# facebookresearch/AudioDec

Hardware: NVIDIA H100
Metric: 48 kHz audio samples/s, encode+quantize+lookup+decode (% HBM roofline in `roofline`) (higher is better)
Workload: dtype f32

## Files before the change

### audiodec_b200/_lib.py

```python
from __future__ import annotations

import ctypes
import os

_HERE = os.path.dirname(os.path.abspath(__file__))
LIB_PATH = os.environ.get("ADEC_LIB_PATH") or os.path.join(_HERE, "lib", "libaudiodec_b200.so")
MAX_STAGES = 8

c_int, c_float, c_void_p, c_char_p = ctypes.c_int, ctypes.c_float, ctypes.c_void_p, ctypes.c_char_p
c_int64 = ctypes.c_int64
_I8 = c_int * MAX_STAGES


class AdecConfig(ctypes.Structure):
    _fields_ = [
        ("model_type", c_int),
        ("input_channels", c_int), ("output_channels", c_int), ("encode_channels", c_int), ("decode_channels", c_int),
        ("code_dim", c_int), ("codebook_num", c_int), ("codebook_size", c_int),
        ("n_enc", c_int), ("enc_ratios", _I8), ("enc_strides", _I8),
        ("n_dec", c_int), ("dec_ratios", _I8), ("dec_strides", _I8),
        ("bias", c_int),
        ("in_channels", c_int), ("out_channels", c_int), ("channels", c_int), ("kernel_size", c_int),
        ("n_up", c_int), ("upsample_scales", _I8), ("upsample_kernel_sizes", _I8),
        ("resblock_kernel_size", c_int),
# ... 9 lines not shown


MODEL_SYMAD, MODEL_HIFIGAN, MODEL_SYMAD_DECODER = 0, 1, 2


class AdecTestOp(ctypes.Structure):
    _fields_ = [
        ("kind", c_int), ("Cin", c_int), ("Cout", c_int), ("K", c_int), ("stride", c_int), ("dil", c_int), ("groups", c_int),
        ("shared_in", c_int), ("pre_act", c_int), ("slope", c_float), ("out_nct", c_int), ("post_tanh", c_int),
        ("w", c_void_p), ("w2", c_void_p), ("bias", c_void_p), ("mean", c_void_p), ("scale", c_void_p),
        ("compute_dtype", c_int),
    ]


TEST_CONV, TEST_RU, TEST_CONVTR, TEST_STEM, TEST_HEAD = 0, 1, 2, 3, 4
TEST_REC = 9

SYMBOLS = {
    "adec_create": (c_int, [ctypes.POINTER(AdecConfig), c_int, ctypes.POINTER(c_void_p)]),
    "adec_destroy": (None, [c_void_p]),
    "adec_last_error": (c_char_p, [c_void_p]),
    "adec_set_tensor": (c_int, [c_void_p, c_char_p, c_void_p, ctypes.POINTER(c_int64), c_int]),
    "adec_finalize": (c_int, [c_void_p]),
    "adec_n_streams": (c_int, [c_void_p]),
    "adec_set_streams": (c_int, [c_void_p, c_int]),
    "adec_reset": (c_int, [c_void_p, c_void_p]),
    "adec_encode": (c_int, [c_void_p, c_void_p, c_int, c_int, c_void_p, c_void_p]),
    "adec_quantize": (c_int, [c_void_p, c_void_p, c_int, c_int, c_void_p, c_void_p]),
    "adec_quantize_ex": (c_int, [c_void_p, c_void_p, c_int, c_int, c_void_p, c_void_p, c_void_p, c_void_p]),
    "adec_quantize_forward": (c_int, [c_void_p, c_void_p, c_int, c_int, c_void_p, c_void_p, c_void_p]),
    "adec_zq_moments": (c_int, [c_void_p, c_void_p, ctypes.POINTER(c_int), c_int, c_void_p, c_void_p, c_void_p]),
# ... 66 lines not shown
```

### audiodec_b200/csrc/adec.cu

```cuda
#include <cuda_runtime.h>

#include <algorithm>
#include <cmath>
#include <cstdarg>
#include <cstdio>
#include <cstring>
#include <map>
#include <memory>
#include <set>
#include <string>
#include <vector>

#include "../../include/audiodec_b200.h"
#include "kernels.cuh"
#include "wg_conv.cuh"
#include <cuda_fp16.h>
#include <cuda_bf16.h>

using namespace adec;

namespace {
thread_local std::string g_create_error;

std::string fmt(const char* f, ...) {
// ... 46 lines not shown
const ConvKernelCfg kConvKernels[] = {
    ADEC_PLAIN(32), ADEC_PLAIN(64), ADEC_PLAIN(96), ADEC_PLAIN(128), ADEC_PLAIN(256),
    {32, 32, 256, 32, true, launch_conv<32, 32, 256, 32, true>},
    {64, 64, 128, 32, true, launch_conv<64, 64, 128, 32, true>},
    {128, 128, 64, 16, true, launch_conv<128, 128, 64, 16, true>},
    {256, 256, 64, 8, true, launch_conv<256, 256, 64, 8, true>},
};

const ConvKernelCfg* find_conv_kernel(int CW, int CO, bool fuse) {
    for (const auto& k : kConvKernels)
        if (k.CW == CW && k.CO == CO && k.fuse == fuse) return &k;
    return nullptr;
}

typedef cudaError_t (*TcPersistFn)(const ConvArgs&, int, int, int, int, int, cudaStream_t);
template <int NT, bool F, int PRE, int PREC, bool BST, bool VL, bool PAIR = false>
cudaError_t launch_wg(const ConvArgs& a, int n_xtiles, int n_ytiles, int n_tiles, int n_ctas, int smem_bytes, cudaStream_t s) {
    static bool configured[64] = {false};
    int dev = 0;
    cudaGetDevice(&dev);
    auto kern = wg_conv_kernel<NT, F, PRE, PREC, BST, VL, PAIR>;
    constexpr int kMaxDyn = 227 * 1024;
    if (dev < 64 && !configured[dev]) {
        cudaError_t e = cudaFuncSetAttribute(kern, cudaFuncAttributeMaxDynamicSharedMemorySize, kMaxDyn);
        if (e != cudaSuccess) return e;
        configured[dev] = true;
    }
    if (smem_bytes > kMaxDyn) return cudaErrorInvalidConfiguration;
    static const bool pdl = [] { const char* e = getenv("ADEC_PDL"); return !e || atoi(e) != 0; }();
    cudaLaunchConfig_t cfg{};
    cfg.gridDim = dim3((unsigned)n_ctas);
    cfg.blockDim = dim3((unsigned)WgCfg<NT, PREC>::THREADS);
    cfg.dynamicSmemBytes = (size_t)smem_bytes;
    cfg.stream = s;
    cudaLaunchAttribute attr[1];
    attr[0].id = cudaLaunchAttributeProgrammaticStreamSerialization;
    attr[0].val.programmaticStreamSerializationAllowed = 1;
    cfg.attrs = attr;
    cfg.numAttrs = pdl ? 1 : 0;
    return cudaLaunchKernelEx(&cfg, kern, a, n_xtiles, n_ytiles, n_tiles);
}
typedef size_t (*TcSmemFn)(int, bool, bool);
typedef int (*TcWbufFn)(int, bool, bool);
template <int NT, bool F, int PRE, int PREC, bool BST>
constexpr TcPersistFn pair_fn() {
    if constexpr (NT == 32 && F && PREC == PREC_F16 && !BST) return launch_wg<NT, F, PRE, PREC, BST, false, true>;
    else return nullptr;
}
struct TcKernelCfg { int NT; bool fuse; int pre, prec; bool bst; int tap_bytes; TcPersistFn pfn, pfn_vl, pfn_pair; TcSmemFn smem; TcWbufFn n_wbuf; };
#define ADEC_TC1(NT, F, PRE, PREC, BST) \
    {NT, F, PRE, PREC, BST, WgCfg<NT, PREC>::TAP_BYTES, launch_wg<NT, F, PRE, PREC, BST, false>, launch_wg<NT, F, PRE, PREC, BST, true>, \
     pair_fn<NT, F, PRE, PREC, BST>(), WgCfg<NT, PREC>::smem_bytes, WgCfg<NT, PREC>::n_wbuf}
#define ADEC_TC_FP32(NT, PREC) \
    ADEC_TC1(NT, true, ACT_ELU, PREC, false), ADEC_TC1(NT, false, ACT_NONE, PREC, false), ADEC_TC1(NT, false, ACT_ELU, PREC, false), \
    ADEC_TC1(NT, false, ACT_LRELU, PREC, false), ADEC_TC1(NT, false, ACT_NORM, PREC, false)
#define ADEC_TC_BF16(NT, BST) \
    ADEC_TC1(NT, false, ACT_NONE, PREC_BF16, BST), ADEC_TC1(NT, false, ACT_LRELU, PREC_BF16, BST), ADEC_TC1(NT, false, ACT_NORM, PREC_BF16, BST), \
    ADEC_TC1(NT, true, ACT_ELU, PREC_BF16, BST), ADEC_TC1(NT, false, ACT_ELU, PREC_BF16, BST)
#define ADEC_TC(NT) ADEC_TC_FP32(NT, PREC_F16), ADEC_TC_FP32(NT, PREC_TF32), ADEC_TC_BF16(NT, false), ADEC_TC_BF16(NT, true)
const TcKernelCfg kTcKernels[] = {ADEC_TC(128), ADEC_TC(64), ADEC_TC(32)};

const TcKernelCfg* find_tc_kernel(int NT, bool fuse, int pre, int prec, bool bst) {
    for (const auto& k : kTcKernels)
        if (k.NT == NT && k.fuse == fuse && k.pre == pre && k.prec == prec && k.bst == bst) return &k;
    return nullptr;
}

// ... 60 lines not shown
    adec_config cfg{};
    int device = 0;
    bool finalized = false;
    std::string err;
    std::map<std::string, HostTensor> tensors;
    std::set<std::string> consumed;
    std::vector<Op> enc_ops, dec_ops;
    int n_streams = 1;
    int st_cap = 1;
    int engine = 2;
    int tc_max_fuse = 128;
    bool bf16 = false;
    bool act_bf16 = false;
    int act_bytes() const { return act_bf16 ? 2 : 4; }
    bool stack_rows = true;
    unsigned long long* d_ktrace = nullptr;
    int ktrace_n = 0;
    int n_sms = 132;
    DevBuf ws[3];
    std::vector<void*> owned;
    float *d_embed = nullptr, *d_e2 = nullptr, *d_codebook = nullptr;
    float *d_mean = nullptr, *d_scale = nullptr;
    int* d_err = nullptr;
    int64_t launches = 0;
    bool profiling = false;
    std::vector<std::pair<cudaEvent_t, cudaEvent_t>> prof_events;
    std::vector<std::string> prof_names;
    std::vector<double> prof_bytes;
    DevBuf hx, hz, hzq, hy;
    DevBuf vl_tab;
// ... 520 lines not shown
                    a.vl_in = vl_in; a.vl_out = vl_out; a.vl_B = rc.B; a.vl_slot = vl_slot;
                } else if (h->stack_rows) {
                    const long long L = (long long)Tout + (long long)(op.Ktaps - 1) * op.dil;
                    const long long stacked = (rc.B * L + TC_TT - 1) / TC_TT;
                    if (stacked * 4 <= (long long)grid.x * rc.B * 3 && rc.B * L < (1ll << 30)) {
                        a.stack_L = (int)L;
                        grid = dim3((unsigned)stacked, grid.y, 1);
                    }
                }
                const bool pair = op.w_pair && !vl && !a.stack_L;
                if (pair) {
                    a.w = op.w_pair;
                    wrows = 2 * pair_rows(op.Ktaps, op.dil);
                    grid.x = (unsigned)((Tout + pair_tt(op.dil) - 1) / pair_tt(op.dil));
                }
                const long long n_tiles = (long long)grid.x * grid.y * grid.z;
                const int n_ctas = (int)std::min<long long>(n_tiles, h->n_sms);
                const size_t psmem = op.tc->smem(wrows, op.fuse, pair);
                a.n_wbuf = op.tc->n_wbuf(wrows, op.fuse, pair);
                if (a.n_wbuf < 1) return h->fail(fmt("%s: window of %d rows does not fit in shared memory", op.name.c_str(), wrows));
                e = (vl ? op.tc->pfn_vl : pair ? op.tc->pfn_pair : op.tc->pfn)(a, (int)grid.x, (int)grid.y, (int)n_tiles, n_ctas, (int)psmem, rc.stream);
                if (h->launch_log)
                    h->launch_log->insert(h->launch_log->end(), {ADEC_TEST_LAUNCH_TC, op.tc->NT, op.tc->fuse, op.tc->pre, op.tc->prec, vl, pair,
                                                                 a.stack_L > 0, op.tc->bst});
            } else {
                const int TT = op.kc->TT;
                dim3 grid((Tout + TT - 1) / TT, op.G * op.n_co_tiles, rc.B);
                e = op.kc->fn(a, grid, TT + (op.Ktaps - 1) * op.dil, rc.stream);
                if (h->launch_log)
                    h->launch_log->insert(h->launch_log->end(), {ADEC_TEST_LAUNCH_FFMA, op.kc->CO, op.kc->fuse, op.pre_act, 0, 0, 0, 0, 0});
            }
        }
        if (h->launch_log && op.kind != OP_CONV)
            h->launch_log->insert(h->launch_log->end(), {op.kind == OP_STEM ? ADEC_TEST_LAUNCH_STEM : ADEC_TEST_LAUNCH_HEAD, 0, 0, op.pre_act,
                                                         0, vl, 0, 0, op.kind == OP_HEAD && h->act_bf16});
        if (e != cudaSuccess) return h->fail(fmt("launch of %s failed: %s", op.name.c_str(), cudaGetErrorString(e)));
        ++h->launches;
        if (h->profiling) {
            cudaEventRecord(ev1, rc.stream);
            h->prof_events.emplace_back(ev0, ev1);
            h->prof_names.push_back(op.name);
            const double cin = op.kind == OP_STEM ? 1 : (double)op.G * op.Cin_eff / std::max(1, op.RG) * (op.shared_in ? 1.0 / op.G : 1.0);
            const double cout = op.kind == OP_HEAD ? 1 : (double)op.G * op.Cout;
            const double eb = h->act_bytes();
            double bytes = eb * nb * (cin * T + cout * Tout);
            if (op.fuse) bytes += eb * nb * (3.0 * cout * Tout);
            else if (op.res_buf >= 0) bytes += eb * nb * cout * Tout;
            h->prof_bytes.push_back(bytes);
        }
        T = Tout * op.up;
// ... 374 lines not shown
    }
    if (cfg->n_enc > ADEC_MAX_STAGES || cfg->n_dec > ADEC_MAX_STAGES || cfg->n_up > ADEC_MAX_STAGES || cfg->n_dil > ADEC_MAX_STAGES) {
        g_create_error = "too many stages";
        return 1;
    }
    auto* h = new adec_handle();
    h->cfg = *cfg;
    h->device = device;
    if (const char* pth = getenv("ADEC_CONV_PATH")) {
        if (!strcmp(pth, "ffma")) h->engine = 0;
        else if (!strcmp(pth, "tf32")) h->engine = 1;
        else if (!strcmp(pth, "f16") || !strcmp(pth, "tc") || !*pth) h->engine = 2;
        else { g_create_error = std::string("ADEC_CONV_PATH must be f16, tf32 or ffma, not ") + pth; delete h; return 1; }
    }
    if (const char* sr = getenv("ADEC_STACK_ROWS")) h->stack_rows = atoi(sr) != 0;
    if (const char* mf = getenv("ADEC_TC_MAXFUSE")) h->tc_max_fuse = atoi(mf);
    if (const char* kt = getenv("ADEC_KTRACE")) {
        if (atoi(kt)) {
            DeviceGuard dgk(device);
            if (cudaMalloc((void**)&h->d_ktrace, 4096 * KT_REC * sizeof(unsigned long long)) == cudaSuccess)
                cudaMemset(h->d_ktrace, 0, 4096 * KT_REC * sizeof(unsigned long long));
        }
    }
    h->bf16 = cfg->compute_dtype == 1 || cfg->compute_dtype == 2;
    h->act_bf16 = cfg->compute_dtype == 2;
    if (cfg->compute_dtype < 0 || cfg->compute_dtype > 2) {
        g_create_error = "compute_dtype must be 0 (fp32), 1 (bf16 operands) or 2 (bf16 operands and activations)";
        delete h;
        return 1;
    }
// ... 963 lines not shown
```

### audiodec_b200/csrc/wg_conv.cuh

```cuda
#pragma once
#include <cuda_bf16.h>
#include <cuda_fp16.h>

#include "kernels.cuh"

namespace adec {

constexpr int TC_TT = 128;
constexpr int TC_CP = 32;
constexpr int TC_MIDP = 128;
constexpr float F16_LO_SCALE = 2048.f;
enum { PREC_BF16 = 1, PREC_TF32 = 2, PREC_F16 = 3 };

__device__ __forceinline__ void fence_async_smem() { asm volatile("fence.proxy.async.shared::cta;" ::: "memory"); }

#ifdef ADEC_PHASES
#define ADEC_PH_START() (ph_t = (uint32_t)clock())
#define ADEC_PH(k) do { const uint32_t ph_now = (uint32_t)clock(); ph[k] += ph_now - ph_t; ph_t = ph_now; } while (0)
#define ADEC_PH_USE(x) (ph_sink += __float_as_uint(x))
#else
#define ADEC_PH_USE(x) ((void)0)
#define ADEC_PH_START() ((void)0)
#define ADEC_PH(k) ((void)0)
#endif
// ... 44 lines not shown
ADEC_WG_N32(PREC_TF32, "k8.f32.tf32.tf32", "")
ADEC_WG_N64(PREC_F16, "k16.f32.f16.f16", ", 0, 0")
ADEC_WG_N64(PREC_BF16, "k16.f32.bf16.bf16", ", 0, 0")
ADEC_WG_N64(PREC_TF32, "k8.f32.tf32.tf32", "")
#undef ADEC_WG_N32
#undef ADEC_WG_N64

template <int NT, int PREC> struct WgCfg {
    static constexpr int EB = PREC == PREC_TF32 ? 4 : 2;
    static constexpr int KBB = TC_CP * EB / 16;
    static constexpr int NPR = PREC == PREC_F16 ? 3 : PREC == PREC_TF32 ? 2 : 1;
    static constexpr int NPL = PREC == PREC_BF16 ? 1 : 2;
    __host__ __device__ static constexpr int tpg(bool fuse) { return PREC == PREC_TF32 || (PREC == PREC_F16 && NT == 32 && fuse) ? 1 : 2; }
    static constexpr int TAP_BYTES = NPR * KBB * NT * 16;
    __host__ __device__ static constexpr int stage_bytes(bool fuse) { return tpg(fuse) * TAP_BYTES; }
    __host__ __device__ static constexpr int mid_bytes(bool pair) { return NPL * (NT * EB / 16) * TC_MIDP * (pair ? 2 : 1) * 16; }
    __host__ __device__ static constexpr int stages(bool fuse, bool pair) { return pair ? 9 : PREC == PREC_TF32 && NT == 128 && fuse ? 1 : NT == 128 ? 2 : 3; }
    __host__ __device__ static constexpr int stage_alloc(bool fuse, bool pair) { return pair ? 2 * TAP_BYTES : stage_bytes(fuse); }
    static constexpr int PW = NT < 64 ? NT : 64;
    static constexpr int NPROD = 96;
    static constexpr int THREADS = 256 + NPROD + 32;
    __host__ __device__ static constexpr int win_pitch(int wrows) { return ((wrows + 1) & ~3) + 2; }
    __host__ __device__ static constexpr int win_bytes(int wrows) { return NPL * KBB * win_pitch(wrows) * 16; }
    static int n_wbuf(int wrows, bool fuse, bool pair) {
        const long long avail = 227 * 1024 - 512 - (long long)stages(fuse, pair) * stage_alloc(fuse, pair) - (fuse ? (long long)mid_bytes(pair) : 0);
        const long long n = avail / win_bytes(wrows);
        return (int)(n > 4 ? 4 : n);
    }
    static size_t smem_bytes(int wrows, bool fuse, bool pair) {
        return 512 + (size_t)stages(fuse, pair) * stage_alloc(fuse, pair) + (size_t)n_wbuf(wrows, fuse, pair) * win_bytes(wrows) +
               (fuse ? (size_t)mid_bytes(pair) : 0);
    }
};

__host__ __device__ constexpr int pair_tt(int dil) { return 2 * dil * (TC_TT / dil); }
__host__ __device__ constexpr int pair_rows(int K, int dil) { return TC_TT + (K - 1) / 2 * dil; }

template <int ACT>
__device__ __forceinline__ float4 apply_act_t(float4 v, float slope) {
    if (ACT == ACT_ELU) { v.x = act_elu(v.x); v.y = act_elu(v.y); v.z = act_elu(v.z); v.w = act_elu(v.w); }
    if (ACT == ACT_LRELU) { v.x = act_lrelu(v.x, slope); v.y = act_lrelu(v.y, slope); v.z = act_lrelu(v.z, slope); v.w = act_lrelu(v.w, slope); }
    return v;
}

__device__ __forceinline__ uint32_t h2_bits(__half2 h) { return *reinterpret_cast<const uint32_t*>(&h); }
__device__ __forceinline__ uint32_t b2_bits(__nv_bfloat162 h) { return *reinterpret_cast<const uint32_t*>(&h); }
// ... 92 lines not shown
                Wgmma<Cfg::PW, PREC>::mma(d, wg_desc(a_hi + t * tap_step + ks * 2u * lbo, lbo), wg_desc(bw + t * B_T + ks * B_KS, B_LBO), acc);
                acc = 1u;
            }
    wg_commit();
    wg_wait0();
    wg_fence_regs(d);
}

template <typename XT>
__device__ __forceinline__ const XT* slot_hist(const ConvArgs& a, int u, int i, int c) {
    const int e = __ldg(a.vl_slot + u);
    const XT* base = reinterpret_cast<const XT*>((e & 1) ? (const void*)a.st_out : (const void*)a.st_in);
    return base + (((e >> 1) * a.P + i) * a.st_ld + c);
}

template <int NT, bool FUSE, int PRE, int PREC, bool BST, bool VL = false, bool PAIR = false>
__global__ void __launch_bounds__(WgCfg<NT, PREC>::THREADS, 1) wg_conv_kernel(const ConvArgs a, int n_xtiles, int n_ytiles, int n_tiles) {
    static_assert(!BST || PREC == PREC_BF16, "bf16 storage is built for the bf16-operand kernels");
    static_assert(!PAIR || (NT == 32 && FUSE && PREC == PREC_F16 && !BST && !VL), "the paired kernel is built for the fused fp16-split RU(32)");
    using Cfg = WgCfg<NT, PREC>;
    using XT = typename std::conditional<BST, __nv_bfloat16, float>::type;
    constexpr int S = Cfg::stages(FUSE, PAIR), CP = TC_CP, TT = TC_TT, KBB = Cfg::KBB, EB = Cfg::EB, TPG = Cfg::tpg(FUSE), PW = Cfg::PW;
    constexpr int NPROD = Cfg::NPROD, WWARP = (256 + NPROD) / 32;
    constexpr int STAGE_BYTES = Cfg::stage_alloc(FUSE, PAIR), TAP_BYTES = Cfg::TAP_BYTES;
    constexpr int NH = NT / PW;
    constexpr int NACC = PAIR ? NT : NT / 2;
    constexpr int MBLK = NT * EB / 16;
    constexpr int MIDP = PAIR ? 2 * TC_MIDP : TC_MIDP;

    extern __shared__ __align__(128) unsigned char smem_raw[];
    uint64_t* b_full = reinterpret_cast<uint64_t*>(smem_raw);
    uint64_t* b_empty = b_full + S;
    uint64_t* w_full = b_empty + S;
    uint64_t* w_empty = w_full + 4;
    unsigned char* bst = smem_raw + 512;
    const int ttile = PAIR ? pair_tt(a.dil) : TT;
    const int wrows = ttile + (a.Ktaps - 1) * a.dil;
    const int prows = PAIR ? pair_rows(a.Ktaps, a.dil) : 0;
    const int wrp = Cfg::win_pitch(PAIR ? 2 * prows : wrows);
    const int win_b = Cfg::win_bytes(PAIR ? 2 * prows : wrows);
    unsigned char* wbuf0 = bst + S * STAGE_BYTES;
    unsigned char* mbuf = wbuf0 + (size_t)a.n_wbuf * win_b;
    auto srow = [&](int m) -> int {
        if constexpr (PAIR) {
            const int blk = m / a.dil;
            return (blk & 1) * prows + (blk >> 1) * a.dil + (m - blk * a.dil);
        } else {
            return m;
        }
    };

// ... 267 lines not shown
        const uint32_t lbo1 = (uint32_t)wrp * 16u, lbo2 = (uint32_t)MIDP * 16u;
        const uint32_t tap_step = (uint32_t)a.dil * 16u;
        constexpr int NPART = PAIR ? PW : PW / 2;
        float racc[NACC];
        float part[NPART];
        float (&part_h)[PW / 2] = *reinterpret_cast<float (*)[PW / 2]>(part);
        int c = 0, wb = 0, wround = 0;
        float vmax = 0.f;
        ADEC_PH_START();
        auto group = [&](uint32_t a_hi, uint32_t a_lo, uint32_t lbo, uint32_t row_off, int ntaps) {
            const int s = c % S;
            mbar_wait(&b_full[s], (c / S) & 1, 300);
            ADEC_PH(PH_WGT);
            const uint32_t bw = bst_u + (uint32_t)s * STAGE_BYTES;
#pragma unroll
            for (int h = 0; h < NH; ++h) {
                wg_group<NT, PREC, TPG>(part_h, a_hi + row_off, a_lo + row_off, lbo, tap_step, ntaps, bw + (uint32_t)h * PW * 16u);
#pragma unroll
                for (int i = 0; i < PW / 2; ++i) racc[h * (PW / 2) + i] = __fadd_rn(racc[h * (PW / 2) + i], part_h[i]);
            }
            ADEC_PH(PH_MMA);
            if (threadIdx.x % 128 == 0) mbar_arrive(&b_empty[s]);
            ++c;
        };
        auto pgroup = [&](uint32_t a_hi, uint32_t a_lo, uint32_t row_off) {
            if constexpr (PAIR) {
                const int s = c % S;
                mbar_wait(&b_full[s], (c / S) & 1, 300);
                ADEC_PH(PH_WGT);
                wg_group<2 * NT, PREC, 1>(part, a_hi + row_off, a_lo + row_off, lbo1, tap_step, 1, bst_u + (uint32_t)s * STAGE_BYTES);
#pragma unroll
                for (int i = 0; i < NACC; ++i) racc[i] = __fadd_rn(racc[i], part[i]);
                ADEC_PH(PH_MMA);
                if (threadIdx.x % 128 == 0) mbar_arrive(&b_empty[s]);
                ++c;
// ... 26 lines not shown
            if (FUSE) {
                const bool ok0 = !PAIR || wrow < ttile / 2, ok8 = !PAIR || wrow + 8 < ttile / 2;
#pragma unroll
                for (int i = 0; i < NACC; i += 4) {
                    const float4 m4 = apply_act_t<PRE>(make_float4(racc[i] * a.w_scale, racc[i + 1] * a.w_scale, racc[i + 2] * a.w_scale, racc[i + 3] * a.w_scale), a.slope);
                    racc[i] = m4.x; racc[i + 1] = m4.y; racc[i + 2] = m4.z; racc[i + 3] = m4.w;
                    if (PAIR) {
                        if (ok0) vmax = fmaxf(vmax, fmaxf(fabsf(m4.x), fabsf(m4.y)));
                        if (ok8) vmax = fmaxf(vmax, fmaxf(fabsf(m4.z), fabsf(m4.w)));
                    } else {
                        vmax = fmaxf(vmax, fmaxf(fmaxf(fabsf(m4.x), fabsf(m4.y)), fmaxf(fabsf(m4.z), fabsf(m4.w))));
                    }
                }
#pragma unroll
                for (int i = 0; i < NACC; i += 2) {
                    const int h = PAIR ? 0 : i / (PW / 2), fi = PAIR ? i : i % (PW / 2);
                    int co = h * PW + 8 * (fi >> 2) + col2, row = wrow + 8 * ((fi >> 1) & 1);
                    if (PAIR) { row += (co / NT) * TC_MIDP; co %= NT; }
                    const int blk = co * EB / 16, off = (co * EB) & 15;
                    unsigned char* hp = mbuf + ((size_t)blk * MIDP + row) * 16 + off;
                    uint2 hi, lo;
                    split2<PREC>(racc[i], racc[i + 1], hi, lo);
                    if (PREC == PREC_TF32) {
                        *reinterpret_cast<uint2*>(hp) = hi;
                        *reinterpret_cast<uint2*>(hp + (size_t)MBLK * MIDP * 16) = lo;
                    } else {
                        *reinterpret_cast<uint32_t*>(hp) = hi.x;
                        if (PREC == PREC_F16) *reinterpret_cast<uint32_t*>(hp + (size_t)MBLK * MIDP * 16) = lo.x;
                    }
                }
                fence_async_smem();
                named_bar_sync(1 + wg, 128);
// ... 9 lines not shown
                        const uint32_t m_hi = mbuf_u + row0_off + (uint32_t)(hh * TC_MIDP * 16);
                        wg_group<NT, PREC, 1>(part_h, m_hi, m_hi + (uint32_t)MBLK * lbo2, lbo2, tap_step, 1, bst_u + (uint32_t)s * STAGE_BYTES);
#pragma unroll
                        for (int i = 0; i < PW / 2; ++i) racc[hh * (PW / 2) + i] = __fadd_rn(racc[hh * (PW / 2) + i], part_h[i]);
                    }
                    if (threadIdx.x % 128 == 0) mbar_arrive(&b_empty[s]);
                    ++c;
                    ADEC_PH(PH_MMA);
                } else {
                    for (int p = 0; p < NT / CP; ++p) {
                        const uint32_t m_hi = mbuf_u + (uint32_t)(p * KBB) * lbo2;
                        group(m_hi, m_hi + (uint32_t)MBLK * lbo2, lbo2, row0_off, 1);
                    }
                }
            }
            constexpr int PB = NT < 128 ? 16 : (PREC == PREC_TF32 && FUSE) || VL ? 4 : 8;
            constexpr int NR = PAIR ? 4 : 2, NCB = NACC / (2 * NR), KB = NCB < PB / NR ? NCB : PB / NR;
            const float oscale = FUSE ? a.w2_scale : a.w_scale;
            const int co0 = co_tile * NT + col2;
            int rt[NR], rbo[NR];
            {
                const int halo = (a.Ktaps - 1) * a.dil;
                int vu = 0, vu_start = 0, vu_next = 0;
                if constexpr (VL) {
                    vu = vl_find(a.vl_out, halo, a.vl_B, j0 + wrow);
                    vu_start = vl_row(a.vl_out, halo, vu);
                    vu_next = vl_row(a.vl_out, halo, vu + 1);
                }
#pragma unroll
                for (int rr = 0; rr < NR; ++rr) {
                    int bo = b, t = j0 + wrow + 8 * rr;
                    bool ok;
                    if constexpr (PAIR) {
                        const int mr = wrow + 8 * (rr & 1), blk = mr / a.dil;
                        t = j0 + blk * 2 * a.dil + (mr - blk * a.dil) + (rr >> 1) * a.dil;
                        ok = mr < ttile / 2 && t < a.Tout;
                    } else if constexpr (VL) {
                        while (vu + 1 < a.vl_B && t >= vu_next) { ++vu; vu_start = vu_next; vu_next = vl_row(a.vl_out, halo, vu + 1); }
                        const int o0 = __ldg(a.vl_out + vu), ml = t - vu_start;
                        ok = ml < __ldg(a.vl_out + vu + 1) - o0;
                        t = o0 + ml;
                    } else {
                        if (a.stack_L) { bo = t / a.stack_L; t -= bo * a.stack_L; }
                        ok = t < a.Tout && bo < a.n_streams;
                    }
                    rt[rr] = ok ? t : -1;
                    rbo[rr] = bo;
                }
            }
#pragma unroll
            for (int k0 = 0; k0 < NCB; k0 += KB) {
                float2 bb[KB], r2[NR][KB];
                if (a.bias) {
#pragma unroll
                    for (int k = 0; k < KB; ++k) {
                        const int co_l = co0 + 8 * (k0 + k);
                        bb[k] = co_l < a.Cout_g ? __ldg(reinterpret_cast<const float2*>(a.bias + g * a.Cout_g + co_l)) : make_float2(0.f, 0.f);
                    }
                }
                if (a.res) {
#pragma unroll
                    for (int rr = 0; rr < NR; ++rr)
#pragma unroll
                        for (int k = 0; k < KB; ++k) {
                            const int t = rt[rr], co_l = co0 + 8 * (k0 + k);
                            r2[rr][k] = t >= 0 && co_l < a.Cout_g
                                            ? ldg2(reinterpret_cast<const XT*>(a.res) + (long long)rbo[rr] * a.res_bs + (long long)t * a.ldr + g * a.r_goff + co_l)
                                            : make_float2(0.f, 0.f);
                        }
                }
#pragma unroll
                for (int rr = 0; rr < NR; ++rr) {
                    const int t = rt[rr], bo = rbo[rr];
                    if (t < 0) continue;
#pragma unroll
                    for (int k = 0; k < KB; ++k) {
                        const int co_l = co0 + 8 * (k0 + k), i = 4 * (k0 + k) + 2 * (rr & 1) + (PW / 2) * (rr >> 1);
                        if (co_l >= a.Cout_g) continue;
                        float v0 = __fmul_rn(racc[i], oscale), v1 = __fmul_rn(racc[i + 1], oscale);
                        if (a.bias) { v0 = __fadd_rn(v0, bb[k].x); v1 = __fadd_rn(v1, bb[k].y); }
                        if (a.res) { v0 = __fadd_rn(r2[rr][k].x, v0); v1 = __fadd_rn(r2[rr][k].y, v1); }
                        vmax = fmaxf(vmax, fmaxf(fabsf(v0), fabsf(v1)));
                        if (a.out_nct) {
                            XT* yp = reinterpret_cast<XT*>(a.y) + (long long)bo * a.y_bs + (long long)(g * a.y_goff + co_l) * a.Tout + t;
                            st1(yp, v0);
                            st1(yp + a.Tout, v1);
                        } else {
                            st2(reinterpret_cast<XT*>(a.y) + (long long)bo * a.y_bs + (long long)t * a.ldy + g * a.y_goff + co_l, v0, v1);
                        }
                    }
                }
            }
            ADEC_PH(PH_EPI);
        }
        if (PREC == PREC_F16 && a.err && !(vmax < 60000.f)) atomicOr(a.err, 2);
    }
#ifdef ADEC_PHASES
    if (a.dbg) {
        if (warp < 8 ? tid % 128 == 0 : warp == WWARP ? lane == 0 : tid == 256) {
            if (ph_sink == 0x7fc00001u) ph[PH_CONV] += 1u;
            for (int k = 0; k < PH_N; ++k)
                if (ph[k]) atomicAdd(a.dbg + 6 + k, (unsigned long long)ph[k]);
        }
        if (blockIdx.x == 0 && tid == 0) {
            a.dbg[3] = (unsigned long long)NT | (FUSE ? 1ull << 8 : 0) | (a.res ? 1ull << 9 : 0) | (PAIR ? 1ull << 10 : 0) |
                       (VL ? 1ull << 11 : 0) | (BST ? 1ull << 12 : 0) | ((unsigned long long)PREC << 13) | ((unsigned long long)a.Ktaps << 16) |
                       ((unsigned long long)a.dil << 24) | ((unsigned long long)(a.n_pieces * CP) << 32) | ((unsigned long long)a.Cout_g << 48);
            a.dbg[4] = (unsigned long long)a.Tout;
            a.dbg[5] = PH_N;
        }
    }
#endif
    if (a.dbg && blockIdx.x == 0 && tid == 0) {
        unsigned long long kt1;
        asm volatile("mov.u64 %0, %%globaltimer;" : "=l"(kt1));
        a.dbg[0] = kt0; a.dbg[1] = kt1; a.dbg[2] = (unsigned long long)(clock64() - kc0);
    }
}

__device__ float g_probe_sink;
template <int NT, int PREC>
// ... 62 lines not shown
```

### include/audiodec_b200.h

```cpp
#ifndef AUDIODEC_B200_H
#define AUDIODEC_B200_H

#include <stdint.h>

#ifdef __cplusplus
extern "C" {
#endif

#define ADEC_MAX_STAGES 8

typedef struct adec_handle adec_handle;

enum adec_model_type {
    ADEC_MODEL_SYMAD = 0,
    ADEC_MODEL_HIFIGAN = 1,
    ADEC_MODEL_SYMAD_DECODER = 2
};

typedef struct adec_config {
    int model_type;
    int input_channels, output_channels, encode_channels, decode_channels;
    int code_dim, codebook_num, codebook_size;
    int n_enc;  int enc_ratios[ADEC_MAX_STAGES];  int enc_strides[ADEC_MAX_STAGES];
    int n_dec;  int dec_ratios[ADEC_MAX_STAGES];  int dec_strides[ADEC_MAX_STAGES];
// ... 83 lines not shown
                            int pre_act, float slope, const float *mean, const float *scale, const void *res, int offline,
                            void *state, void *y);

enum { ADEC_TEST_CONV = 0, ADEC_TEST_RU = 1, ADEC_TEST_CONVTR = 2, ADEC_TEST_STEM = 3, ADEC_TEST_HEAD = 4 };
typedef struct adec_test_op {
    int kind;
    int Cin, Cout;
    int K, stride, dil, groups, shared_in;
    int pre_act;
    float slope;
    int out_nct;
    int post_tanh;
    const float *w, *w2, *bias, *mean, *scale;
    int compute_dtype;
} adec_test_op;
enum { ADEC_TEST_REC = 9, ADEC_TEST_LAUNCH_TC = 0, ADEC_TEST_LAUNCH_FFMA = 1, ADEC_TEST_LAUNCH_STEM = 2, ADEC_TEST_LAUNCH_HEAD = 3 };
int adec_test_conv_op(int device, const adec_test_op *op, int mode, int n_calls, int B, int n_streams, const int *lengths,
                      const int *streams, const float *x, const float *res, float *state, float *y, int *launched, int max_launched,
                      int *range_flag);

int adec_record_launches(adec_handle *h, int enable);
int adec_launch_records(const adec_handle *h, int *out, int max_records);

#ifdef __cplusplus
}
#endif
#endif
```

Baseline: 179.1 million.

## Add two-row-block variant of fused NT=64 fp16 residual-unit conv kernel

Result: faster. 182.8 million, median of 6 (+2.1%).

```diff
diff --git a/audiodec_b200/_lib.py b/audiodec_b200/_lib.py
--- a/audiodec_b200/_lib.py
+++ b/audiodec_b200/_lib.py
@@ -47,7 +47,7 @@
 
 
 TEST_CONV, TEST_RU, TEST_CONVTR, TEST_STEM, TEST_HEAD = 0, 1, 2, 3, 4
-TEST_REC = 9
+TEST_REC = 10
 
 SYMBOLS = {
     "adec_create": (c_int, [ctypes.POINTER(AdecConfig), c_int, ctypes.POINTER(c_void_p)]),
diff --git a/audiodec_b200/csrc/adec.cu b/audiodec_b200/csrc/adec.cu
--- a/audiodec_b200/csrc/adec.cu
+++ b/audiodec_b200/csrc/adec.cu
@@ -84,12 +84,12 @@
 }
 
 typedef cudaError_t (*TcPersistFn)(const ConvArgs&, int, int, int, int, int, cudaStream_t);
-template <int NT, bool F, int PRE, int PREC, bool BST, bool VL, bool PAIR = false>
+template <int NT, bool F, int PRE, int PREC, bool BST, bool VL, bool PAIR = false, int RB = 1>
 cudaError_t launch_wg(const ConvArgs& a, int n_xtiles, int n_ytiles, int n_tiles, int n_ctas, int smem_bytes, cudaStream_t s) {
     static bool configured[64] = {false};
     int dev = 0;
     cudaGetDevice(&dev);
-    auto kern = wg_conv_kernel<NT, F, PRE, PREC, BST, VL, PAIR>;
+    auto kern = wg_conv_kernel<NT, F, PRE, PREC, BST, VL, PAIR, RB>;
     constexpr int kMaxDyn = 227 * 1024;
     if (dev < 64 && !configured[dev]) {
         cudaError_t e = cudaFuncSetAttribute(kern, cudaFuncAttributeMaxDynamicSharedMemorySize, kMaxDyn);
@@ -110,17 +110,22 @@
     cfg.numAttrs = pdl ? 1 : 0;
     return cudaLaunchKernelEx(&cfg, kern, a, n_xtiles, n_ytiles, n_tiles);
 }
-typedef size_t (*TcSmemFn)(int, bool, bool);
-typedef int (*TcWbufFn)(int, bool, bool);
+typedef size_t (*TcSmemFn)(int, bool, bool, bool);
+typedef int (*TcWbufFn)(int, bool, bool, bool);
 template <int NT, bool F, int PRE, int PREC, bool BST>
 constexpr TcPersistFn pair_fn() {
     if constexpr (NT == 32 && F && PREC == PREC_F16 && !BST) return launch_wg<NT, F, PRE, PREC, BST, false, true>;
     else return nullptr;
 }
-struct TcKernelCfg { int NT; bool fuse; int pre, prec; bool bst; int tap_bytes; TcPersistFn pfn, pfn_vl, pfn_pair; TcSmemFn smem; TcWbufFn n_wbuf; };
+template <int NT, bool F, int PRE, int PREC, bool BST>
+constexpr TcPersistFn rb_fn() {
+    if constexpr (NT == 64 && F && PREC == PREC_F16 && !BST) return launch_wg<NT, F, PRE, PREC, BST, false, false, 2>;
+    else return nullptr;
+}
+struct TcKernelCfg { int NT; bool fuse; int pre, prec; bool bst; int tap_bytes; TcPersistFn pfn, pfn_vl, pfn_pair, pfn_rb; TcSmemFn smem; TcWbufFn n_wbuf; };
 #define ADEC_TC1(NT, F, PRE, PREC, BST) \
     {NT, F, PRE, PREC, BST, WgCfg<NT, PREC>::TAP_BYTES, launch_wg<NT, F, PRE, PREC, BST, false>, launch_wg<NT, F, PRE, PREC, BST, true>, \
-     pair_fn<NT, F, PRE, PREC, BST>(), WgCfg<NT, PREC>::smem_bytes, WgCfg<NT, PREC>::n_wbuf}
+     pair_fn<NT, F, PRE, PREC, BST>(), rb_fn<NT, F, PRE, PREC, BST>(), WgCfg<NT, PREC>::smem_bytes, WgCfg<NT, PREC>::n_wbuf}
 #define ADEC_TC_FP32(NT, PREC) \
     ADEC_TC1(NT, true, ACT_ELU, PREC, false), ADEC_TC1(NT, false, ACT_NONE, PREC, false), ADEC_TC1(NT, false, ACT_ELU, PREC, false), \
     ADEC_TC1(NT, false, ACT_LRELU, PREC, false), ADEC_TC1(NT, false, ACT_NORM, PREC, false)
@@ -211,6 +216,7 @@
     bool act_bf16 = false;
     int act_bytes() const { return act_bf16 ? 2 : 4; }
     bool stack_rows = true;
+    bool row_blocks = true;
     unsigned long long* d_ktrace = nullptr;
     int ktrace_n = 0;
     int n_sms = 132;
@@ -761,26 +767,32 @@
                     wrows = 2 * pair_rows(op.Ktaps, op.dil);
                     grid.x = (unsigned)((Tout + pair_tt(op.dil) - 1) / pair_tt(op.dil));
                 }
+                const bool rb = op.tc->pfn_rb && h->row_blocks && !vl && !a.stack_L;
+                if (rb) {
+                    wrows = 2 * TC_TT + (op.Ktaps - 1) * op.dil;
+                    grid.x = (unsigned)((Tout + 2 * TC_TT - 1) / (2 * TC_TT));
+                }
                 const long long n_tiles = (long long)grid.x * grid.y * grid.z;
                 const int n_ctas = (int)std::min<long long>(n_tiles, h->n_sms);
-                const size_t psmem = op.tc->smem(wrows, op.fuse, pair);
-                a.n_wbuf = op.tc->n_wbuf(wrows, op.fuse, pair);
+                const size_t psmem = op.tc->smem(wrows, op.fuse, pair, rb);
+                a.n_wbuf = op.tc->n_wbuf(wrows, op.fuse, pair, rb);
                 if (a.n_wbuf < 1) return h->fail(fmt("%s: window of %d rows does not fit in shared memory", op.name.c_str(), wrows));
-                e = (vl ? op.tc->pfn_vl : pair ? op.tc->pfn_pair : op.tc->pfn)(a, (int)grid.x, (int)grid.y, (int)n_tiles, n_ctas, (int)psmem, rc.stream);
+                e = (vl ? op.tc->pfn_vl : pair ? op.tc->pfn_pair : rb ? op.tc->pfn_rb : op.tc->pfn)(a, (int)grid.x, (int)grid.y, (int)n_tiles,
+                                                                                                     n_ctas, (int)psmem, rc.stream);
                 if (h->launch_log)
                     h->launch_log->insert(h->launch_log->end(), {ADEC_TEST_LAUNCH_TC, op.tc->NT, op.tc->fuse, op.tc->pre, op.tc->prec, vl, pair,
-                                                                 a.stack_L > 0, op.tc->bst});
+                                                                 a.stack_L > 0, op.tc->bst, rb});
             } else {
                 const int TT = op.kc->TT;
                 dim3 grid((Tout + TT - 1) / TT, op.G * op.n_co_tiles, rc.B);
                 e = op.kc->fn(a, grid, TT + (op.Ktaps - 1) * op.dil, rc.stream);
                 if (h->launch_log)
-                    h->launch_log->insert(h->launch_log->end(), {ADEC_TEST_LAUNCH_FFMA, op.kc->CO, op.kc->fuse, op.pre_act, 0, 0, 0, 0, 0});
+                    h->launch_log->insert(h->launch_log->end(), {ADEC_TEST_LAUNCH_FFMA, op.kc->CO, op.kc->fuse, op.pre_act, 0, 0, 0, 0, 0, 0});
             }
         }
         if (h->launch_log && op.kind != OP_CONV)
             h->launch_log->insert(h->launch_log->end(), {op.kind == OP_STEM ? ADEC_TEST_LAUNCH_STEM : ADEC_TEST_LAUNCH_HEAD, 0, 0, op.pre_act,
-                                                         0, vl, 0, 0, op.kind == OP_HEAD && h->act_bf16});
+                                                         0, vl, 0, 0, op.kind == OP_HEAD && h->act_bf16, 0});
         if (e != cudaSuccess) return h->fail(fmt("launch of %s failed: %s", op.name.c_str(), cudaGetErrorString(e)));
         ++h->launches;
         if (h->profiling) {
@@ -1185,6 +1197,7 @@
         else { g_create_error = std::string("ADEC_CONV_PATH must be f16, tf32 or ffma, not ") + pth; delete h; return 1; }
     }
     if (const char* sr = getenv("ADEC_STACK_ROWS")) h->stack_rows = atoi(sr) != 0;
+    if (const char* rb = getenv("ADEC_ROW_BLOCKS")) h->row_blocks = atoi(rb) != 0;
     if (const char* mf = getenv("ADEC_TC_MAXFUSE")) h->tc_max_fuse = atoi(mf);
     if (const char* kt = getenv("ADEC_KTRACE")) {
         if (atoi(kt)) {
diff --git a/audiodec_b200/csrc/wg_conv.cuh b/audiodec_b200/csrc/wg_conv.cuh
--- a/audiodec_b200/csrc/wg_conv.cuh
+++ b/audiodec_b200/csrc/wg_conv.cuh
@@ -82,7 +82,7 @@
     __host__ __device__ static constexpr int tpg(bool fuse) { return PREC == PREC_TF32 || (PREC == PREC_F16 && NT == 32 && fuse) ? 1 : 2; }
     static constexpr int TAP_BYTES = NPR * KBB * NT * 16;
     __host__ __device__ static constexpr int stage_bytes(bool fuse) { return tpg(fuse) * TAP_BYTES; }
-    __host__ __device__ static constexpr int mid_bytes(bool pair) { return NPL * (NT * EB / 16) * TC_MIDP * (pair ? 2 : 1) * 16; }
+    __host__ __device__ static constexpr int mid_bytes(bool two) { return NPL * (NT * EB / 16) * TC_MIDP * (two ? 2 : 1) * 16; }
     __host__ __device__ static constexpr int stages(bool fuse, bool pair) { return pair ? 9 : PREC == PREC_TF32 && NT == 128 && fuse ? 1 : NT == 128 ? 2 : 3; }
     __host__ __device__ static constexpr int stage_alloc(bool fuse, bool pair) { return pair ? 2 * TAP_BYTES : stage_bytes(fuse); }
     static constexpr int PW = NT < 64 ? NT : 64;
@@ -90,14 +90,14 @@
     static constexpr int THREADS = 256 + NPROD + 32;
     __host__ __device__ static constexpr int win_pitch(int wrows) { return ((wrows + 1) & ~3) + 2; }
     __host__ __device__ static constexpr int win_bytes(int wrows) { return NPL * KBB * win_pitch(wrows) * 16; }
-    static int n_wbuf(int wrows, bool fuse, bool pair) {
-        const long long avail = 227 * 1024 - 512 - (long long)stages(fuse, pair) * stage_alloc(fuse, pair) - (fuse ? (long long)mid_bytes(pair) : 0);
+    static int n_wbuf(int wrows, bool fuse, bool pair, bool rb) {
+        const long long avail = 227 * 1024 - 512 - (long long)stages(fuse, pair) * stage_alloc(fuse, pair) - (fuse ? (long long)mid_bytes(pair || rb) : 0);
         const long long n = avail / win_bytes(wrows);
         return (int)(n > 4 ? 4 : n);
     }
-    static size_t smem_bytes(int wrows, bool fuse, bool pair) {
-        return 512 + (size_t)stages(fuse, pair) * stage_alloc(fuse, pair) + (size_t)n_wbuf(wrows, fuse, pair) * win_bytes(wrows) +
-               (fuse ? (size_t)mid_bytes(pair) : 0);
+    static size_t smem_bytes(int wrows, bool fuse, bool pair, bool rb) {
+        return 512 + (size_t)stages(fuse, pair) * stage_alloc(fuse, pair) + (size_t)n_wbuf(wrows, fuse, pair, rb) * win_bytes(wrows) +
+               (fuse ? (size_t)mid_bytes(pair || rb) : 0);
     }
 };
 
@@ -220,19 +220,23 @@
     return base + (((e >> 1) * a.P + i) * a.st_ld + c);
 }
 
-template <int NT, bool FUSE, int PRE, int PREC, bool BST, bool VL = false, bool PAIR = false>
+template <int NT, bool FUSE, int PRE, int PREC, bool BST, bool VL = false, bool PAIR = false, int RB = 1>
 __global__ void __launch_bounds__(WgCfg<NT, PREC>::THREADS, 1) wg_conv_kernel(const ConvArgs a, int n_xtiles, int n_ytiles, int n_tiles) {
     static_assert(!BST || PREC == PREC_BF16, "bf16 storage is built for the bf16-operand kernels");
     static_assert(!PAIR || (NT == 32 && FUSE && PREC == PREC_F16 && !BST && !VL), "the paired kernel is built for the fused fp16-split RU(32)");
+    static_assert(RB == 1 || (RB == 2 && NT == 64 && FUSE && PREC == PREC_F16 && !BST && !VL && !PAIR),
+                  "the row-block kernel is built for the fused NT = 64 fp16-split unit");
     using Cfg = WgCfg<NT, PREC>;
     using XT = typename std::conditional<BST, __nv_bfloat16, float>::type;
     constexpr int S = Cfg::stages(FUSE, PAIR), CP = TC_CP, TT = TC_TT, KBB = Cfg::KBB, EB = Cfg::EB, TPG = Cfg::tpg(FUSE), PW = Cfg::PW;
     constexpr int NPROD = Cfg::NPROD, WWARP = (256 + NPROD) / 32;
     constexpr int STAGE_BYTES = Cfg::stage_alloc(FUSE, PAIR), TAP_BYTES = Cfg::TAP_BYTES;
     constexpr int NH = NT / PW;
-    constexpr int NACC = PAIR ? NT : NT / 2;
+    constexpr int NBA = NT / 2;
+    constexpr int NACC = PAIR ? NT : RB * NBA;
     constexpr int MBLK = NT * EB / 16;
-    constexpr int MIDP = PAIR ? 2 * TC_MIDP : TC_MIDP;
+    constexpr int MIDP = PAIR || RB == 2 ? 2 * TC_MIDP : TC_MIDP;
+    constexpr uint32_t RB_OFF = (uint32_t)TC_TT * 16u;
 
     extern __shared__ __align__(128) unsigned char smem_raw[];
     uint64_t* b_full = reinterpret_cast<uint64_t*>(smem_raw);
@@ -240,7 +244,7 @@
     uint64_t* w_full = b_empty + S;
     uint64_t* w_empty = w_full + 4;
     unsigned char* bst = smem_raw + 512;
-    const int ttile = PAIR ? pair_tt(a.dil) : TT;
+    const int ttile = PAIR ? pair_tt(a.dil) : RB * TT;
     const int wrows = ttile + (a.Ktaps - 1) * a.dil;
     const int prows = PAIR ? pair_rows(a.Ktaps, a.dil) : 0;
     const int wrp = Cfg::win_pitch(PAIR ? 2 * prows : wrows);
@@ -538,11 +542,15 @@
             ADEC_PH(PH_WGT);
             const uint32_t bw = bst_u + (uint32_t)s * STAGE_BYTES;
 #pragma unroll
-            for (int h = 0; h < NH; ++h) {
-                wg_group<NT, PREC, TPG>(part_h, a_hi + row_off, a_lo + row_off, lbo, tap_step, ntaps, bw + (uint32_t)h * PW * 16u);
-#pragma unroll
-                for (int i = 0; i < PW / 2; ++i) racc[h * (PW / 2) + i] = __fadd_rn(racc[h * (PW / 2) + i], part_h[i]);
-            }
+            for (int rb = 0; rb < RB; ++rb)
+#pragma unroll
+                for (int h = 0; h < NH; ++h) {
+                    const uint32_t ro = row_off + (uint32_t)rb * RB_OFF;
+                    wg_group<NT, PREC, TPG>(part_h, a_hi + ro, a_lo + ro, lbo, tap_step, ntaps, bw + (uint32_t)h * PW * 16u);
+                    const int i0 = rb * NBA + h * (PW / 2);
+#pragma unroll
+                    for (int i = 0; i < PW / 2; ++i) racc[i0 + i] = __fadd_rn(racc[i0 + i], part_h[i]);
+                }
             ADEC_PH(PH_MMA);
             if (threadIdx.x % 128 == 0) mbar_arrive(&b_empty[s]);
             ++c;
@@ -599,8 +607,9 @@
                 }
 #pragma unroll
                 for (int i = 0; i < NACC; i += 2) {
-                    const int h = PAIR ? 0 : i / (PW / 2), fi = PAIR ? i : i % (PW / 2);
-                    int co = h * PW + 8 * (fi >> 2) + col2, row = wrow + 8 * ((fi >> 1) & 1);
+                    const int rb = PAIR ? 0 : i / NBA, ib = i - rb * NBA;
+                    const int h = PAIR ? 0 : ib / (PW / 2), fi = PAIR ? i : ib % (PW / 2);
+                    int co = h * PW + 8 * (fi >> 2) + col2, row = wrow + 8 * ((fi >> 1) & 1) + rb * TC_TT;
                     if (PAIR) { row += (co / NT) * TC_MIDP; co %= NT; }
                     const int blk = co * EB / 16, off = (co * EB) & 15;
                     unsigned char* hp = mbuf + ((size_t)blk * MIDP + row) * 16 + off;
@@ -640,79 +649,123 @@
                     }
                 }
             }
-            constexpr int PB = NT < 128 ? 16 : (PREC == PREC_TF32 && FUSE) || VL ? 4 : 8;
-            constexpr int NR = PAIR ? 4 : 2, NCB = NACC / (2 * NR), KB = NCB < PB / NR ? NCB : PB / NR;
-            const float oscale = FUSE ? a.w2_scale : a.w_scale;
-            const int co0 = co_tile * NT + col2;
-            int rt[NR], rbo[NR];
-            {
-                const int halo = (a.Ktaps - 1) * a.dil;
-                int vu = 0, vu_start = 0, vu_next = 0;
-                if constexpr (VL) {
-                    vu = vl_find(a.vl_out, halo, a.vl_B, j0 + wrow);
-                    vu_start = vl_row(a.vl_out, halo, vu);
-                    vu_next = vl_row(a.vl_out, halo, vu + 1);
-                }
-#pragma unroll
-                for (int rr = 0; rr < NR; ++rr) {
-                    int bo = b, t = j0 + wrow + 8 * rr;
-                    bool ok;
-                    if constexpr (PAIR) {
-                        const int mr = wrow + 8 * (rr & 1), blk = mr / a.dil;
-                        t = j0 + blk * 2 * a.dil + (mr - blk * a.dil) + (rr >> 1) * a.dil;
-                        ok = mr < ttile / 2 && t < a.Tout;
-                    } else if constexpr (VL) {
-                        while (vu + 1 < a.vl_B && t >= vu_next) { ++vu; vu_start = vu_next; vu_next = vl_row(a.vl_out, halo, vu + 1); }
-                        const int o0 = __ldg(a.vl_out + vu), ml = t - vu_start;
-                        ok = ml < __ldg(a.vl_out + vu + 1) - o0;
-                        t = o0 + ml;
-                    } else {
-                        if (a.stack_L) { bo = t / a.stack_L; t -= bo * a.stack_L; }
-                        ok = t < a.Tout && bo < a.n_streams;
-                    }
-                    rt[rr] = ok ? t : -1;
-                    rbo[rr] = bo;
-                }
-            }
-#pragma unroll
-            for (int k0 = 0; k0 < NCB; k0 += KB) {
-                float2 bb[KB], r2[NR][KB];
-                if (a.bias) {
-#pragma unroll
-                    for (int k = 0; k < KB; ++k) {
-                        const int co_l = co0 + 8 * (k0 + k);
-                        bb[k] = co_l < a.Cout_g ? __ldg(reinterpret_cast<const float2*>(a.bias + g * a.Cout_g + co_l)) : make_float2(0.f, 0.f);
-                    }
-                }
-                if (a.res) {
-#pragma unroll
-                    for (int rr = 0; rr < NR; ++rr)
+            if constexpr (RB == 2) {
+                const float oscale = a.w2_scale;
+                float2 bb[NBA / 4];
+#pragma unroll
+                for (int k = 0; k < NBA / 4; ++k) {
+                    const int co_l = co_tile * NT + 8 * k + col2;
+                    bb[k] = a.bias && co_l < a.Cout_g ? __ldg(reinterpret_cast<const float2*>(a.bias + g * a.Cout_g + co_l)) : make_float2(0.f, 0.f);
+                }
+                named_bar_sync(1 + wg, 128);
+#pragma unroll
+                for (int i = 0; i < NACC; i += 2) {
+                    const int rb = i / NBA, fi = i - rb * NBA;
+                    const int col = 8 * (fi >> 2) + col2, row = wrow + 8 * ((fi >> 1) & 1) + rb * TC_TT, slab = col >> 2;
+                    float v0 = __fmul_rn(racc[i], oscale), v1 = __fmul_rn(racc[i + 1], oscale);
+                    if (a.bias) { v0 = __fadd_rn(v0, bb[fi >> 2].x); v1 = __fadd_rn(v1, bb[fi >> 2].y); }
+                    *reinterpret_cast<float2*>(mbuf + ((size_t)slab * MIDP + (row ^ (slab & 7))) * 16 + (col & 3) * 4) = make_float2(v0, v1);
+                }
+                __syncwarp();
+                constexpr int NS = 8;
+                const int slab = lane & 15, cg = co_tile * NT + 4 * slab;
+                const bool col_ok = cg < a.Cout_g;
+#pragma unroll
+                for (int rb = 0; rb < RB; ++rb) {
+                    const int row0 = rb * TC_TT + 64 * wg + 16 * (warp & 3) + (lane >> 4);
+                    float4 r4[NS];
+#pragma unroll
+                    for (int s = 0; s < NS; ++s) {
+                        const int t = j0 + row0 + 2 * s;
+                        r4[s] = a.res && col_ok && t < a.Tout
+                                    ? ldg4(reinterpret_cast<const XT*>(a.res) + (long long)b * a.res_bs + (long long)t * a.ldr + g * a.r_goff + cg)
+                                    : make_float4(0.f, 0.f, 0.f, 0.f);
+                    }
+#pragma unroll
+                    for (int s = 0; s < NS; ++s) {
+                        const int row = row0 + 2 * s, t = j0 + row;
+                        if (!col_ok || t >= a.Tout) continue;
+                        float4 v = *reinterpret_cast<const float4*>(mbuf + ((size_t)slab * MIDP + (row ^ (slab & 7))) * 16);
+                        if (a.res) { v.x = __fadd_rn(r4[s].x, v.x); v.y = __fadd_rn(r4[s].y, v.y); v.z = __fadd_rn(r4[s].z, v.z); v.w = __fadd_rn(r4[s].w, v.w); }
+                        vmax = fmaxf(vmax, fmaxf(fmaxf(fabsf(v.x), fabsf(v.y)), fmaxf(fabsf(v.z), fabsf(v.w))));
+                        st4(reinterpret_cast<XT*>(a.y) + (long long)b * a.y_bs + (long long)t * a.ldy + g * a.y_goff + cg, v);
+                    }
+                }
+            } else {
+                constexpr int PB = NT < 128 ? 16 : (PREC == PREC_TF32 && FUSE) || VL ? 4 : 8;
+                constexpr int NR = PAIR ? 4 : 2, NCB = NACC / (2 * NR), KB = NCB < PB / NR ? NCB : PB / NR;
+                const float oscale = FUSE ? a.w2_scale : a.w_scale;
+                const int co0 = co_tile * NT + col2;
+                int rt[NR], rbo[NR];
+                {
+                    const int halo = (a.Ktaps - 1) * a.dil;
+                    int vu = 0, vu_start = 0, vu_next = 0;
+                    if constexpr (VL) {
+                        vu = vl_find(a.vl_out, halo, a.vl_B, j0 + wrow);
+                        vu_start = vl_row(a.vl_out, halo, vu);
+                        vu_next = vl_row(a.vl_out, halo, vu + 1);
+                    }
+#pragma unroll
+                    for (int rr = 0; rr < NR; ++rr) {
+                        int bo = b, t = j0 + wrow + 8 * rr;
+                        bool ok;
+                        if constexpr (PAIR) {
+                            const int mr = wrow + 8 * (rr & 1), blk = mr / a.dil;
+                            t = j0 + blk * 2 * a.dil + (mr - blk * a.dil) + (rr >> 1) * a.dil;
+                            ok = mr < ttile / 2 && t < a.Tout;
+                        } else if constexpr (VL) {
+                            while (vu + 1 < a.vl_B && t >= vu_next) { ++vu; vu_start = vu_next; vu_next = vl_row(a.vl_out, halo, vu + 1); }
+                            const int o0 = __ldg(a.vl_out + vu), ml = t - vu_start;
+                            ok = ml < __ldg(a.vl_out + vu + 1) - o0;
+                            t = o0 + ml;
+                        } else {
+                            if (a.stack_L) { bo = t / a.stack_L; t -= bo * a.stack_L; }
+                            ok = t < a.Tout && bo < a.n_streams;
+                        }
+                        rt[rr] = ok ? t : -1;
+                        rbo[rr] = bo;
+                    }
+                }
+#pragma unroll
+                for (int k0 = 0; k0 < NCB; k0 += KB) {
+                    float2 bb[KB], r2[NR][KB];
+                    if (a.bias) {
 #pragma unroll
                         for (int k = 0; k < KB; ++k) {
-                            const int t = rt[rr], co_l = co0 + 8 * (k0 + k);
-                            r2[rr][k] = t >= 0 && co_l < a.Cout_g
-                                            ? ldg2(reinterpret_cast<const XT*>(a.res) + (long long)rbo[rr] * a.res_bs + (long long)t * a.ldr + g * a.r_goff + co_l)
-                                            : make_float2(0.f, 0.f);
+                            const int co_l = co0 + 8 * (k0 + k);
+                            bb[k] = co_l < a.Cout_g ? __ldg(reinterpret_cast<const float2*>(a.bias + g * a.Cout_g + co_l)) : make_float2(0.f, 0.f);
                         }
-                }
-#pragma unroll
-                for (int rr = 0; rr < NR; ++rr) {
-                    const int t = rt[rr], bo = rbo[rr];
-                    if (t < 0) continue;
-#pragma unroll
-                    for (int k = 0; k < KB; ++k) {
-                        const int co_l = co0 + 8 * (k0 + k), i = 4 * (k0 + k) + 2 * (rr & 1) + (PW / 2) * (rr >> 1);
-                        if (co_l >= a.Cout_g) continue;
-                        float v0 = __fmul_rn(racc[i], oscale), v1 = __fmul_rn(racc[i + 1], oscale);
-                        if (a.bias) { v0 = __fadd_rn(v0, bb[k].x); v1 = __fadd_rn(v1, bb[k].y); }
-                        if (a.res) { v0 = __fadd_rn(r2[rr][k].x, v0); v1 = __fadd_rn(r2[rr][k].y, v1); }
-                        vmax = fmaxf(vmax, fmaxf(fabsf(v0), fabsf(v1)));
-                        if (a.out_nct) {
-                            XT* yp = reinterpret_cast<XT*>(a.y) + (long long)bo * a.y_bs + (long long)(g * a.y_goff + co_l) * a.Tout + t;
-                            st1(yp, v0);
-                            st1(yp + a.Tout, v1);
-                        } else {
-                            st2(reinterpret_cast<XT*>(a.y) + (long long)bo * a.y_bs + (long long)t * a.ldy + g * a.y_goff + co_l, v0, v1);
+                    }
+                    if (a.res) {
+#pragma unroll
+                        for (int rr = 0; rr < NR; ++rr)
+#pragma unroll
+                            for (int k = 0; k < KB; ++k) {
+                                const int t = rt[rr], co_l = co0 + 8 * (k0 + k);
+                                r2[rr][k] = t >= 0 && co_l < a.Cout_g
+                                                ? ldg2(reinterpret_cast<const XT*>(a.res) + (long long)rbo[rr] * a.res_bs + (long long)t * a.ldr + g * a.r_goff + co_l)
+                                                : make_float2(0.f, 0.f);
+                            }
+                    }
+#pragma unroll
+                    for (int rr = 0; rr < NR; ++rr) {
+                        const int t = rt[rr], bo = rbo[rr];
+                        if (t < 0) continue;
+#pragma unroll
+                        for (int k = 0; k < KB; ++k) {
+                            const int co_l = co0 + 8 * (k0 + k), i = 4 * (k0 + k) + 2 * (rr & 1) + (PW / 2) * (rr >> 1);
+                            if (co_l >= a.Cout_g) continue;
+                            float v0 = __fmul_rn(racc[i], oscale), v1 = __fmul_rn(racc[i + 1], oscale);
+                            if (a.bias) { v0 = __fadd_rn(v0, bb[k].x); v1 = __fadd_rn(v1, bb[k].y); }
+                            if (a.res) { v0 = __fadd_rn(r2[rr][k].x, v0); v1 = __fadd_rn(r2[rr][k].y, v1); }
+                            vmax = fmaxf(vmax, fmaxf(fabsf(v0), fabsf(v1)));
+                            if (a.out_nct) {
+                                XT* yp = reinterpret_cast<XT*>(a.y) + (long long)bo * a.y_bs + (long long)(g * a.y_goff + co_l) * a.Tout + t;
+                                st1(yp, v0);
+                                st1(yp + a.Tout, v1);
+                            } else {
+                                st2(reinterpret_cast<XT*>(a.y) + (long long)bo * a.y_bs + (long long)t * a.ldy + g * a.y_goff + co_l, v0, v1);
+                            }
                         }
                     }
                 }
@@ -730,7 +783,8 @@
         }
         if (blockIdx.x == 0 && tid == 0) {
             a.dbg[3] = (unsigned long long)NT | (FUSE ? 1ull << 8 : 0) | (a.res ? 1ull << 9 : 0) | (PAIR ? 1ull << 10 : 0) |
-                       (VL ? 1ull << 11 : 0) | (BST ? 1ull << 12 : 0) | ((unsigned long long)PREC << 13) | ((unsigned long long)a.Ktaps << 16) |
+                       (VL ? 1ull << 11 : 0) | (BST ? 1ull << 12 : 0) | ((unsigned long long)PREC << 13) | (RB == 2 ? 1ull << 15 : 0) |
+                       ((unsigned long long)a.Ktaps << 16) |
                        ((unsigned long long)a.dil << 24) | ((unsigned long long)(a.n_pieces * CP) << 32) | ((unsigned long long)a.Cout_g << 48);
             a.dbg[4] = (unsigned long long)a.Tout;
             a.dbg[5] = PH_N;
diff --git a/include/audiodec_b200.h b/include/audiodec_b200.h
--- a/include/audiodec_b200.h
+++ b/include/audiodec_b200.h
@@ -121,7 +121,7 @@
     const float *w, *w2, *bias, *mean, *scale;
     int compute_dtype;
 } adec_test_op;
-enum { ADEC_TEST_REC = 9, ADEC_TEST_LAUNCH_TC = 0, ADEC_TEST_LAUNCH_FFMA = 1, ADEC_TEST_LAUNCH_STEM = 2, ADEC_TEST_LAUNCH_HEAD = 3 };
+enum { ADEC_TEST_REC = 10, ADEC_TEST_LAUNCH_TC = 0, ADEC_TEST_LAUNCH_FFMA = 1, ADEC_TEST_LAUNCH_STEM = 2, ADEC_TEST_LAUNCH_HEAD = 3 };
 int adec_test_conv_op(int device, const adec_test_op *op, int mode, int n_calls, int B, int n_streams, const int *lengths,
                       const int *streams, const float *x, const float *res, float *state, float *y, int *launched, int max_launched,
                       int *range_flag);
```
